# Ekumen-OS/beluga

Hardware: AMD Instinct MI355X
Metric: MCL update cycles/sec (motion+sensor+resample), N particles x 1080 beams (higher is better)
Workload: dtype f64; 1 GPU; BASELINE configs[1]: 1M particles/GPU, 1080-beam LikelihoodFieldModel, 4000x4000@5cm grid (seed 42), DifferentialDriveModel, multinomial resample every cycle; particles_per_gpu=1000000, particles_total=1000000, beams=1080, grid=4000x4000@0.05, parallelism=1 GPU

## Files before the change

### beluga_amd/csrc/context.hip

```cpp
#include <hip/hip_runtime.h>
#include <dlfcn.h>

#include <algorithm>
#include <cctype>
#include <atomic>
#include <chrono>
#include <thread>
#include <cmath>
#include <cstdio>
#include <cstring>
#include <limits>
#include <new>
#include <numeric>
#include <optional>
#include <string>
#include <unordered_set>
#include <map>
#include <vector>

#include "beluga_mcl.h"
#include "cluster_host.h"
#include "cycle_host.h"
#include "kernels.h"
#include "landmark_host.h"
// ... 1054 lines not shown
  const double* d_total = ctx->d_scalars.ptr + kSlotCdfTotal;
  uint64_t result = max_p;
  if (a.min_particles >= max_p) {
    ra.first_candidate = 0;
    ra.count = max_p;
    ra.out_offset = 0;
    if (opt.with_estimate) {
      MCL_HIP(ctx, ctx->d_est_partials.ensure(static_cast<size_t>(9) * ((max_p + 1023) / 1024)));
      Completion done{};
      const bool spin = ctx->tuning.cycle_spin > 0 || (ctx->tuning.cycle_spin < 0 && max_p >= 262144);
      ctx->done_armed = spin && ctx->profile <= 1 && opt.estimate_enqueued;
      if (ctx->done_armed) {
        done.d_ticket = reinterpret_cast<unsigned long long*>(ctx->d_scalars.ptr + kSlotDoneTicket);
        done.host_flag = reinterpret_cast<unsigned long long*>(ctx->hd_scalars + kSlotDoneWord);
        done.seq = ++ctx->done_seq;
      }
      const bool noise_in_draw = ctx->tuning.noise_ahead == 1 && max_p > 65536 && max_p <= 2000000 &&
                                 ctx->d_noise.ensure(3 * static_cast<size_t>(max_p)) == hipSuccess;
      const bool noise_ahead = ctx->done_armed && ctx->tuning.noise_ahead == 2 && max_p > 65536 && max_p <= 2000000 &&
                               ctx->d_noise.ensure(3 * static_cast<size_t>(max_p)) == hipSuccess;
      KeyFrame ahead_frame{};
      const bool order_keys = noise_in_draw && ctx->done_armed && ctx->tuning.order_ahead != 0 && max_p < (1ull << 32) && ctx->wants_ordering() &&
                              ctx->predict_key_frame(&ctx->last_sampler, &ahead_frame, 2);
      launch_resample_draw_and_estimate(ctx->stream, ctx->cur(), ctx->cdf_tree(), d_total, ctx->other(), ra, gv, fc, hp,
                                        ctx->facts.pivot()[0], ctx->facts.pivot()[1], ctx->d_est_partials.ptr, ctx->d_scalars.ptr + kSlotEstimate,
                                        ctx->hd_scalars + kSlotEstimate, ctx->done_armed ? &done : nullptr,
                                        ((ctx->tuning.draw_fold == 2 || (ctx->tuning.draw_fold == 1 && max_p <= 65536)) && ctx->d_scan_state.ptr)
                                            ? reinterpret_cast<unsigned int*>(ctx->d_scan_state.ptr + 4)
                                            : nullptr,
                                        noise_in_draw ? ctx->d_noise.ptr : nullptr, max_p, ctx->cfg.shard_offset, step + 1,
                                        order_keys ? ctx->sort_scratch().keys : nullptr, &ctx->last_sampler, &ahead_frame);
      if (noise_ahead) launch_noise_ahead(ctx->stream, ctx->cfg.seed, step + 1, ctx->cfg.shard_offset, max_p, ctx->d_noise.ptr);
      if (noise_ahead || noise_in_draw) ctx->facts.noise_ahead_recorded(step + 1, max_p, ctx->cfg.shard_offset, ctx->cfg.seed);
      if (order_keys) {
        const SortScratch sort = ctx->sort_scratch();
        launch_order_ahead(ctx->stream, max_p, &sort);
        ctx->facts.order_ahead_recorded(step + 1, max_p, ctx->key_layout());
        ctx->order_sampler = ctx->last_sampler;
      }
      if (opt.estimate_enqueued) *opt.estimate_enqueued = true;
    } else {
      launch_resample_draw(ctx->stream, ctx->cur(), ctx->cdf_tree(), d_total, ctx->other(), ra, gv, fc, hp, nullptr);
    }
    MCL_HIP(ctx, hipGetLastError());
  } else {
    MCL_REQUIRE(ctx, max_p < 0xFFFFFFFFull, "max_particles too large for KLD resampling");
    if (const mcl_status s = kld_begin(ctx)) return s;
    uint64_t chunk = std::max<uint64_t>(a.min_particles + 1, 1ull << 16);
    while (ctx->kld_pos < max_p) {
      const uint64_t pos = ctx->kld_pos;
      const uint64_t cnt = std::min(chunk, max_p - pos);
      if (const mcl_status s = kld_grow_table(ctx, pos + cnt)) return s;
      ra.first_candidate = pos;
      ra.count = cnt;
      ra.out_offset = pos;
      launch_resample_draw(ctx->stream, ctx->cur(), ctx->cdf_tree(), d_total, ctx->other(), ra, gv, fc, hp, ctx->d_hashes.ptr);
      uint64_t first_fail = ~0ull;
      if (const mcl_status s = kld_process(ctx, cnt, &first_fail)) return s;
      if (first_fail != ~0ull) {
// ... 948 lines not shown
      MCL_HIP(ctx, hipStreamCreateWithFlags(&ctx->stream, hipStreamNonBlocking));
      ctx->own_stream = true;
    }
    const uint64_t cap = cfg->shard_capacity ? cfg->shard_capacity : cfg->amcl.max_particles;
    if (const mcl_status s = ensure_capacity(ctx, cap)) return s;
    MCL_HIP(ctx, ctx->d_scalars.ensure(kScalarSlots));
    MCL_HIP(ctx, hipMemsetAsync(ctx->d_scalars.ptr, 0, kScalarSlots * sizeof(double), ctx->stream));
    MCL_HIP(ctx, hipHostMalloc(reinterpret_cast<void**>(&ctx->h_scalars), kScalarSlots * sizeof(double), hipHostMallocMapped));
    std::memset(ctx->h_scalars, 0, kScalarSlots * sizeof(double));
    MCL_HIP(ctx, hipHostGetDevicePointer(reinterpret_cast<void**>(&ctx->hd_scalars), ctx->h_scalars, 0));
    MCL_HIP(ctx, ctx->d_kld_scalars.ensure(8));
    MCL_HIP(ctx, hipMemsetAsync(ctx->d_kld_scalars.ptr, 0, 8 * sizeof(unsigned long long), ctx->stream));
    MCL_HIP(ctx, hipHostMalloc(reinterpret_cast<void**>(&ctx->h_kld_scalars), 8 * sizeof(unsigned long long)));
    for (auto& pair : ctx->ev)
      for (auto& e : pair) MCL_HIP(ctx, hipEventCreate(&e));
    MCL_HIP(ctx, hipEventCreateWithFlags(&ctx->points_event, hipEventDisableTiming));
    MCL_HIP(ctx, configure_device_kernels());
    {
      int count = 0;
      if (hipDeviceGetAttribute(&count, hipDeviceAttributeMultiprocessorCount, ctx->device) != hipSuccess || count <= 0) count = 256;
      ctx->tuning.device_cus = count;
    }
    for (const char* name : {"lf_variant", "lf_fast", "lf_table", "lf_patch", "lf_dispersed", "lf_far_tiles", "key_layout", "lf_loose_below", "lf_small_particles", "device_policy",
                             "sort_min_particles", "beam_sort_min_particles", "field_build", "key_curve", "key_warp", "key_bits_xy", "lf_margin", "lf_split", "lf_queue_grid", "shard_pad_permille", "lf_queue", "lf_ends_first", "beam_free_ahead", "beam_sectors", "lf_weight_sums", "beam_table", "cycle_spin", "scan_fused", "draw_fold", "lf_unit_weights", "small_fused", "norm_store", "noise_ahead", "order_ahead", "lf_far_beams_per_wave", "batch_cluster_fused"}) {
      std::string env = "BELUGA_MCL_";
      for (const char* c = name; *c; ++c) env += static_cast<char>(std::toupper(static_cast<unsigned char>(*c)));
      if (const char* v = std::getenv(env.c_str())) {
        if (std::string(name) == "lf_table") (void)mcl_set_option(ctx, name, std::string(v) == "cube" ? 1 : std::atoi(v));
        else (void)mcl_set_option(ctx, name, std::atoi(v));
      }
    }
    return MCL_OK;
  };
  st = init();
  if (st != MCL_OK) {
    g_create_error = ctx->error;
    mcl_destroy(ctx);
    return st;
  }
  *out = ctx;
  return MCL_OK;
}

void mcl_destroy(mcl_ctx* ctx) {
  if (!ctx || ctx->batch) return;
  drop_pending_map(ctx);
  (void)hipSetDevice(ctx->device);
// ... 1374 lines not shown
      t.shard_pad_permille = before;
      return s;
    }
  }
  else if (key == "lf_queue_grid") t.lf_queue_grid = static_cast<int>(std::clamp<int64_t>(value, 0, 1 << 20));
  else if (key == "cycle_spin") t.cycle_spin = value < 0 ? -1 : (value ? 1 : 0);
  else if (key == "beam_table") {
    t.beam_table = value ? 1 : 0;
    if (!t.beam_table && ctx->beam_table_ready) {
      if (bind_device(ctx) == MCL_OK && hipStreamSynchronize(ctx->stream) == hipSuccess) {
        ctx->d_beam_table.release();
        ctx->beam_table_ready = false;
      }
    }
  }
  else if (key == "lf_weight_sums") t.lf_weight_sums = value ? 1 : 0;
  else if (key == "scan_fused") t.scan_fused = static_cast<int>(std::clamp<int64_t>(value, 0, 2));
  else if (key == "draw_fold") t.draw_fold = static_cast<int>(std::clamp<int64_t>(value, 0, 2));
  else if (key == "lf_unit_weights") t.lf_unit_weights = value ? 1 : 0;
  else if (key == "small_fused") t.small_fused = value ? 1 : 0;
  else if (key == "batch_cluster_fused") t.batch_cluster_fused = value ? 1 : 0;
  else if (key == "norm_store") t.norm_store = value ? 1 : 0;
  else if (key == "order_ahead") t.order_ahead = value ? 1 : 0;
  else if (key == "noise_ahead") t.noise_ahead = static_cast<int>(std::clamp<int64_t>(value, 0, 2));
  else if (key == "lf_split") t.lf_split = static_cast<int>(value & 3);
  else if (key == "sort_min_particles") t.sort_min_particles = static_cast<int>(std::clamp<int64_t>(value, 0, 1ll << 30));
  else if (key == "beam_sort_min_particles") t.beam_sort_min_particles = static_cast<int>(std::clamp<int64_t>(value, 0, 1ll << 30));
  else return fail(ctx, MCL_ERR_INVALID_ARGUMENT, "mcl_set_option: unknown option " + key);
  return MCL_OK;
}

mcl_status mcl_get_counter(mcl_ctx* ctx, const char* name, uint64_t* value) {
  if (!ctx || !name || !value) return MCL_ERR_INVALID_ARGUMENT;
  const std::string key(name);
  if (key == "lf_fast_launches") *value = ctx->lf_fast_launches;
  else if (key == "lf_patch_launches") *value = ctx->lf_patch_launches;
  else if (key == "lf_queue_launches") *value = ctx->lf_queue_launches;
  else if (key == "lf_beams_launches") *value = ctx->lf_beams_launches;
  else if (key == "lf_far_launches") *value = ctx->lf_far_launches;
  else if (key == "lf_far_beams_launches") *value = ctx->lf_far_beams_launches;
  else if (key == "small_tail_launches") *value = ctx->small_tail_launches;
  else if (key == "estimate_repivots") *value = ctx->estimate_repivots;
  else if (key == "lf_far_tiles") *value = ctx->map->far_tiles;
  else if (key == "noise_ahead_used") *value = ctx->noise_ahead_used;
  else if (key == "order_ahead_used") *value = ctx->order_ahead_used;
  else if (key == "order_ahead_missed") *value = ctx->order_ahead_missed;
// ... 343 lines not shown
```

### beluga_amd/csrc/cycle_types.h

```cpp
#pragma once

#include <algorithm>
#include <cstdint>

namespace mcl {

struct DiffDriveSampler {
  int kind;
  double m1, s1, mt, st, m2, s2;
  double first_c, first_s;
};

enum LfVariant : int {
  kLfWavePerParticle = 0,
  kLfLanePerParticle = 1,
  kLfSortedLanes = 2,
  kLfBeamLanes = 3
};

struct Tuning {
  int lf_variant = kLfSortedLanes;
  int lf_fast = -1;
  int lf_table = 0;
  int lf_patch = 1;
// ... 6 lines not shown
  int lf_far_tiles = 1;
  int key_layout = -1;
  int lf_small_particles = 65536;
  int field_build = 0;
  int key_curve = 1;
  int key_warp = 1;
  int key_bits_xy = 0;
  int cycle_spin = -1;
  int beam_table = 1;
  int lf_weight_sums = 1;
  int lf_split = 3;
  int lf_margin = 1;
  int beam_free_ahead = 1;
  int lf_queue_grid = 0;
  int device_cus = 0;
  int shard_pad_permille = 1063;
  int lf_ends_first = 1;
  int beam_sectors = 1;
  int lf_queue = 1;
  int scan_fused = 1;
  int draw_fold = 1;
  int noise_ahead = 1;
  int order_ahead = 1;
  int norm_store = 0;
  int batch_cluster_fused = 1;
  int small_fused = 1;
  int lf_unit_weights = 1;
};

struct KeyFrame {
  double cx, cy;
  double c0, s0;
  float inv_x, inv_y;
  float inv_t, t_off;
  uint32_t layout;
  uint32_t bits_xy;
};

inline bool lf_set_is_small(uint64_t n, const Tuning& t) {
  return n < static_cast<uint64_t>(std::max(t.sort_min_particles, t.lf_small_particles));
}

}
```

### beluga_amd/csrc/kernels.h

```cpp
#pragma once
#include <hip/hip_runtime.h>

#include <algorithm>
#include <cstdint>

#include "batch_host.h"
#include "cycle_types.h"
#include "se2.h"
#include "sensor_records.h"

namespace mcl {

struct Particles {
  double4* pose;
  double* w;
};

struct FieldView {
  const float* data;
  uint32_t W, H;
  double inv_resolution;
  Pose2 world_to_field;
  float unknown_value;
  const double* cube;
// ... 168 lines not shown
  }
}
struct SortScratch {
  uint32_t* keys;
  uint32_t* perm;
  uint32_t* table;
  uint32_t* totals;
  unsigned long long* keyidx;
  double* bbox;
  KeyFrame* frame;
  double* partial;
};
constexpr uint32_t kLfMaxSegments = 16;
constexpr uint64_t kLfSegmentedBelow = 262144;

void launch_propagate(hipStream_t st, Particles p, uint64_t n, DiffDriveSampler smp, uint64_t seed, uint32_t step,
                      uint64_t index_offset, const double* scan_src = nullptr, double* scan_dst = nullptr, uint32_t scan_doubles = 0,
                      const SortScratch* sort = nullptr, const KeyFrame* frame = nullptr, const double* normals_ahead = nullptr,
                      uint64_t normals_stride = 0);
void launch_noise_ahead(hipStream_t st, uint64_t seed, uint32_t step, uint64_t index_offset, uint64_t n, double* d_normals);
void launch_pull_scan(hipStream_t st, const double* scan_src, double* scan_dst, uint32_t scan_doubles);
void launch_order_particles(hipStream_t st, Particles p, uint64_t n, const SortScratch* sort, const KeyFrame* frame, bool keys_ready,
                            uint32_t layout = 0);
void launch_order_ahead(hipStream_t st, uint64_t n, const SortScratch* sort);
struct PatchStats {
  unsigned long long* device;
  unsigned long long* mirror;
  uint32_t loose_below;
  uint32_t isotropic_margin;
  uint32_t split_patches;
  double* weight_sums;
  unsigned int* arrivals;
};
struct LfReweightArgs {
  Particles p;
  uint64_t n;
  FieldView f;
  const double* d_points;
  uint32_t B;
  const SortScratch* sort;
  bool patches, beams;
  bool dispersed;
  double scan_cells;
  bool unit_weights;
  PatchStats stats;
};
enum class LfKernel { kNone, kPatch, kPatchQueue, kFarBeams, kPaletteFar, kPaletteFast, kPaletteExact, kSortedCube, kSortedField, kBeams, kIndexOrder };
// ... 141 lines not shown
  unsigned long long done_seq;
};
SmallTailArgs small_tail_args(const SmallTail& t);
bool small_tail_fits(uint64_t n, uint64_t max_particles);

struct BatchItem {
  Particles p;
  uint64_t n;
  DiffDriveSampler smp;
  uint64_t seed;
  uint32_t step;
  uint64_t index_offset;
  const double* scan_src;
  double* scan_dst;
  uint32_t scan_doubles;
  FieldView f;
  uint32_t B;
  SmallTailArgs tail;
  uint32_t first_propagate_block, first_reweight_block;
};
void launch_batch_cycle(hipStream_t st, const BatchItem* d_items, const BatchGrid& grid);
void launch_resample_draw(hipStream_t st, Particles src, CdfTree cdf, const double* d_total, Particles dst,
                          ResampleArgs a, GridView g, FreeCells fc, HashParams hp, unsigned long long* d_hashes);
void launch_resample_draw_and_estimate(hipStream_t st, Particles src, CdfTree cdf, const double* d_total, Particles dst, ResampleArgs a,
                                       GridView g, FreeCells fc, HashParams hp, double pivot_x, double pivot_y, double* d_partials,
                                       double* d_sums, double* host_mirror, const Completion* done = nullptr,
                                       unsigned int* fold_ticket = nullptr, double* normals_ahead = nullptr, uint64_t normals_stride = 0,
                                       uint64_t normals_index_offset = 0, uint32_t normals_step = 0, uint32_t* keys_ahead = nullptr,
                                       const DiffDriveSampler* predicted = nullptr, const KeyFrame* frame_ahead = nullptr);
void launch_resample_targets(hipStream_t st, uint64_t seed, uint32_t step, double p, double total, uint64_t first_slot,
                             uint64_t count, uint64_t n_free, double* d_targets, const double* d_plan = nullptr);
struct RecoveryPolicy;
void launch_shard_plan(hipStream_t st, const double* d_stats, uint32_t world, uint64_t n_total, double* d_sums, double* sums_mirror,
                       const RecoveryPolicy& policy, double* d_intervals, double* d_plan);
void launch_route_targets(hipStream_t st, const double* d_targets, uint64_t count, const double* d_ends, const double* d_offsets,
                          uint32_t world, uint32_t self_rank, uint8_t* d_dest, uint32_t* d_block_hist, uint32_t* d_chunk_sum,
                          uint32_t* d_chunk_off, double* d_send_targets, uint32_t* d_order, long long* d_counts, uint32_t pad_capacity = 0,
                          double* d_overflow = nullptr);
void launch_gather_by_cdf_aos(hipStream_t st, Particles src, CdfTree cdf, const double* d_targets, uint64_t m,
                              double* d_out);
void launch_commit_routed(hipStream_t st, Particles dst, uint64_t seed, uint32_t step, uint64_t first_slot, uint64_t count,
                          const double* d_replies, const uint32_t* d_order, const double* d_targets, GridView g, FreeCells fc);
void launch_commit_injected(hipStream_t st, Particles dst, uint64_t seed, uint32_t step, uint64_t first_slot, uint64_t count,
                            const double* d_targets, GridView g, FreeCells fc);
void launch_finish_candidates(hipStream_t st, uint64_t seed, uint32_t step, uint64_t first_slot, uint64_t count, const double* d_replies,
                              const uint32_t* d_order, const double* d_targets, GridView g, FreeCells fc, HashParams hp,
                              double* d_states, unsigned long long* d_hashes);
struct KldTable {
  unsigned long long* keys;
  unsigned int* first;
  uint64_t capacity;
};
// ... 82 lines not shown
```

### beluga_amd/csrc/kernels.hip

```cpp
#include "device_common.hpp"


namespace mcl {
namespace {

constexpr uint32_t kKeyBitsXY = 6, kKeyBitsTheta = 8, kKeyBits = 2 * kKeyBitsXY + kKeyBitsTheta;
constexpr uint32_t kDigitBits = 10;
static_assert((1u << kDigitBits) == kSortDigits && kKeyBits == 2 * kDigitBits, "two passes of one digit each");
__device__ __forceinline__ uint32_t spread3(uint32_t v) {
  v &= 0x3FF;
  v = (v | (v << 16)) & 0x030000FF;
  v = (v | (v << 8)) & 0x0300F00F;
  v = (v | (v << 4)) & 0x030C30C3;
  v = (v | (v << 2)) & 0x09249249;
  return v;
}
__device__ __forceinline__ uint32_t spread2(uint32_t v) {
  v &= 0x3F;
  v = (v | (v << 4)) & 0x30F;
  v = (v | (v << 2)) & 0x333;
  v = (v | (v << 1)) & 0x555;
  return v;
}
__device__ __forceinline__ int unit_bin(float u, int bins) {
// ... 1447 lines not shown
      const uint32_t key = order_key(p.pose[i], kf);
      keys[i] = key;
      atomicAdd(&hist[key >> kDigitBits], 1u);
    }
  }
  __syncthreads();
  for (uint32_t d = threadIdx.x; d < kSortDigits; d += kWide) table[static_cast<size_t>(d) * nblocks + blockIdx.x] = hist[d];
}

__global__ __launch_bounds__(kWide) void k_key_hist(const uint32_t* __restrict__ keys, uint64_t n, uint32_t* __restrict__ table, uint32_t nblocks) {
  __shared__ uint32_t hist[kSortDigits];
  for (uint32_t d = threadIdx.x; d < kSortDigits; d += kWide) hist[d] = 0;
  __syncthreads();
  const uint64_t base = static_cast<uint64_t>(blockIdx.x) * kChunk;
#pragma unroll
  for (int k = 0; k < kChunk / kWide; ++k) {
    const uint64_t i = base + k * kWide + threadIdx.x;
    if (i < n) atomicAdd(&hist[keys[i] >> kDigitBits], 1u);
  }
  __syncthreads();
  for (uint32_t d = threadIdx.x; d < kSortDigits; d += kWide) table[static_cast<size_t>(d) * nblocks + blockIdx.x] = hist[d];
}

__global__ __launch_bounds__(kBlock) void k_row_scan(uint32_t* __restrict__ table, uint32_t nblocks, uint32_t* __restrict__ totals) {
  const uint32_t d = blockIdx.x * (kBlock / 64) + (threadIdx.x >> 6), lane = threadIdx.x & 63;
  uint32_t* row = table + static_cast<size_t>(d) * nblocks;
  uint32_t carry = 0;
  for (uint32_t start = 0; start < nblocks; start += 64) {
    const uint32_t b = start + lane;
    const uint32_t v = b < nblocks ? row[b] : 0u;
    uint32_t incl = v;
#pragma unroll
    for (int o = 1; o < 64; o <<= 1) {
      const uint32_t up = __shfl_up(incl, o);
      if (lane >= static_cast<uint32_t>(o)) incl += up;
    }
    if (b < nblocks) row[b] = carry + incl - v;
    carry += __shfl(incl, 63);
  }
  if (lane == 0) totals[d] = carry;
}
template <int T>
__device__ __forceinline__ void digit_bases(const uint32_t* __restrict__ totals, uint32_t* s_base, uint32_t* s_wave ) {
  constexpr int kPer = kSortDigits / T;
  const uint32_t lane = threadIdx.x & 63, wave = threadIdx.x >> 6;
  uint32_t v[kPer], sum = 0;
#pragma unroll
  for (int k = 0; k < kPer; ++k) {
    v[k] = totals[threadIdx.x * kPer + k];
    sum += v[k];
  }
  uint32_t incl = sum;
#pragma unroll
  for (int o = 1; o < 64; o <<= 1) {
    const uint32_t up = __shfl_up(incl, o);
    if (lane >= static_cast<uint32_t>(o)) incl += up;
  }
  if (lane == 63) s_wave[wave] = incl;
  __syncthreads();
  uint32_t prefix = incl - sum;
  for (uint32_t q = 0; q < wave; ++q) prefix += s_wave[q];
#pragma unroll
  for (int k = 0; k < kPer; ++k) {
// ... 294 lines not shown
      if (base + e < n) a[base + e] = lds[chunk_slot(e)];
    }
  }
}

__global__ __launch_bounds__(kBlock) void k_chunk_sum(const double* __restrict__ w, uint64_t n, double* __restrict__ partials) {
  __shared__ double scratch[kBlock / 64];
  __shared__ double s_items[kChunkPadded];
  double x[kItems];
  chunk_items_load(w, n, s_items, x);
  double v[1] = {0.0};
#pragma unroll
  for (int k = 0; k < kItems; ++k) v[0] += x[k];
  block_reduce<1>(v, scratch);
  if (threadIdx.x == 0) partials[blockIdx.x] = v[0];
}

__device__ __forceinline__ double row_total(const double* __restrict__ row, uint32_t count, double* scratch ) {
  double v[1] = {0.0};
  for (uint32_t b = threadIdx.x; b < count; b += kBlock) v[0] += row[b];
  block_reduce<1>(v, scratch);
  return v[0];
}
__global__ __launch_bounds__(kBlock) void k_final_rows(const double* __restrict__ partials, uint32_t count, uint32_t stride,
                                                       double* __restrict__ out, double* __restrict__ host_mirror, Completion done) {
  __shared__ double scratch[kBlock / 64];
  const uint32_t k = blockIdx.x;
  const double total = row_total(partials + static_cast<size_t>(k) * stride, count, scratch);
  if (threadIdx.x == 0) {
    out[k] = total;
    if (host_mirror) host_mirror[k] = total;
    if (done.host_flag) {
      __threadfence_system();
      const unsigned long long ticket = atomicAdd(done.d_ticket, 1ull);
      if (ticket % gridDim.x == gridDim.x - 1) {
        __threadfence_system();
        __hip_atomic_store(done.host_flag, done.seq, __ATOMIC_RELEASE, __HIP_MEMORY_SCOPE_SYSTEM);
      }
    }
  }
}

__global__ __launch_bounds__(kBlock) void k_normalize(double* __restrict__ w, uint64_t n, const double* __restrict__ d_factor,
                                                      double* __restrict__ chunk_sum, double* __restrict__ chunk_sumsq,
                                                      const double* __restrict__ sum_partials, uint32_t sum_count,
                                                      double* __restrict__ d_sum_out, double* __restrict__ sum_mirror, int store_weights) {
  __shared__ double scratch[(kBlock / 64) * 2];
  __shared__ double s_factor;
  if (sum_partials) {
    double t[1] = {0.0};
    for (uint32_t b = threadIdx.x; b < sum_count; b += kBlock) t[0] += sum_partials[b];
    block_reduce<1>(t, scratch);
    if (threadIdx.x == 0) {
      s_factor = t[0];
      if (blockIdx.x == 0) {
        d_sum_out[0] = t[0];
        if (sum_mirror) sum_mirror[0] = t[0];
      }
    }
    __syncthreads();
  }
  const double factor = sum_partials ? s_factor : *d_factor;
  const bool skip = fabs(factor - 1.0) < DBL_EPSILON;
// ... 515 lines not shown
  return s;
}

__device__ __forceinline__ bool intersperse_here(const RngWords& r, uint64_t j, double p, uint64_t n_free) {
  return j > 0 && p > 0.0 && rng_uniform32(r.w[2]) < p && n_free > 0;
}

constexpr int kDrawBlock = 1024;
constexpr uint32_t kDrawStageMax = 4608;
struct DrawFold {
  unsigned int* ticket{nullptr};
  double* out{nullptr};
  double* host_mirror{nullptr};
  Completion done{};
};
struct DrawNormals {
  double* normals{nullptr};
  uint64_t stride{0};
  uint64_t index_offset{0};
  uint32_t step{0};
  uint32_t* keys{nullptr};
  DiffDriveSampler predicted{};
  KeyFrame frame{};
};
__device__ __forceinline__ double4 predicted_pose_f32(const Pose2& p, const DiffDriveSampler& m, float z0, float z1, float z2) {
  const float c = static_cast<float>(p.r.c), s = static_cast<float>(p.r.s);
  float turn, ahead, left, dir_c, dir_s;
  if (m.kind == 1) {
    turn = z0 * static_cast<float>(m.s1) + static_cast<float>(m.m1);
    ahead = z1 * static_cast<float>(m.st) + static_cast<float>(m.mt);
    left = -(z2 * static_cast<float>(m.s2));
    dir_c = static_cast<float>(m.first_c);
    dir_s = static_cast<float>(m.first_s);
  } else if (m.kind == 2) {
    turn = z0 * 0.02f;
    ahead = z1 * 0.02f;
    left = z2 * 0.02f;
    dir_c = 1.f;
    dir_s = 0.f;
  } else {
    const float r1 = z0 * static_cast<float>(m.s1) + static_cast<float>(m.m1);
    turn = r1 + z2 * static_cast<float>(m.s2) + static_cast<float>(m.m2);
    ahead = z1 * static_cast<float>(m.st) + static_cast<float>(m.mt);
    left = 0.f;
    dir_c = __cosf(r1);
    dir_s = __sinf(r1);
  }
  const float hc = c * dir_c - s * dir_s, hs = s * dir_c + c * dir_s;
  const float tc = __cosf(turn), ts = __sinf(turn);
  return double4{static_cast<double>(c * tc - s * ts), static_cast<double>(s * tc + c * ts),
                 p.x + static_cast<double>(ahead * hc - left * hs), p.y + static_cast<double>(ahead * hs + left * hc)};
}
template <bool kEstimate>
__global__ __launch_bounds__(kDrawBlock) __attribute__((amdgpu_waves_per_eu(8, 8))) void k_resample_draw(Particles src, CdfTree cdf, const double* __restrict__ d_total,
                                                              Particles dst, ResampleArgs a, GridView g, FreeCells fc, HashParams hp,
                                                              unsigned long long* __restrict__ hashes, double pivot_x, double pivot_y,
                                                              double* __restrict__ est_partials, uint32_t est_stride, int first_staged,
                                                              uint32_t staged_doubles, DrawFold fold, DrawNormals ahead) {
  extern __shared__ __attribute__((aligned(16))) unsigned char smem[];
  double* staged = reinterpret_cast<double*>(smem);
  __shared__ double scratch[kEstimate ? (kDrawBlock / 64) * 9 : 1];
  if (first_staged < cdf.depth) {
    const double* from = cdf.levels + cdf.offset[first_staged];
    for (uint32_t k = threadIdx.x; k < staged_doubles; k += kDrawBlock) staged[k] = from[k];
  }
  __syncthreads();
  const uint64_t t = static_cast<uint64_t>(blockIdx.x) * kDrawBlock + threadIdx.x;
  double v[9] = {0, 0, 0, 0, 0, 0, 0, 0, 0};
  const uint64_t j = a.first_candidate + t;
  const RngWords r = rng_draw(a.seed, a.step, kRngResample, j);
  const double p_random = a.d_random_state_probability ? *a.d_random_state_probability : a.random_state_probability;
  const bool intersperse = t < a.count && intersperse_here(r, j, p_random, fc.count);
  uint64_t idx = 0;
  if (a.n_in >= 2) {
    const double target = (t < a.count && !intersperse) ? rng_uniform53(r.w[0], r.w[1]) * (*d_total) : 0.0;
    idx = cdf_tree_lower_bound_staged(cdf, staged, first_staged, target);
  }
  if (t < a.count) {
    Pose2 s;
    if (intersperse) {
      s = random_free_state(a.seed, a.step, j, g, fc);
    } else {
      s = load_pose(src, idx);
    }
    const uint64_t o = a.out_offset + t;
    store_pose(dst, o, s);
    dst.w[o] = 1.0;
    if (hashes) hashes[o] = spatial_hash(s, hp);
    if (ahead.normals) {
      const double4 z = propagation_normals(a.seed, ahead.step, ahead.index_offset + o);
      ahead.normals[o] = z.x;
      ahead.normals[ahead.stride + o] = z.y;
      ahead.normals[2 * ahead.stride + o] = z.z;
      if (ahead.keys)
        ahead.keys[o] = order_key(predicted_pose_f32(s, ahead.predicted, static_cast<float>(z.x), static_cast<float>(z.y), static_cast<float>(z.z)),
                                  ahead.frame);
    }
    if (kEstimate) {
      const double dx = s.x - pivot_x, dy = s.y - pivot_y;
      v[0] = 1.0;
      v[1] = 1.0;
      v[2] = s.r.c;
      v[3] = s.r.s;
      v[4] = dx;
      v[5] = dy;
      v[6] = dx * dx;
      v[7] = dx * dy;
      v[8] = dy * dy;
    }
  }
  if (kEstimate) {
    block_reduce<9, kDrawBlock>(v, scratch);
    if (fold.ticket == nullptr) {
      if (threadIdx.x == 0) {
#pragma unroll
        for (int k = 0; k < 9; ++k) est_partials[static_cast<size_t>(k) * est_stride + blockIdx.x] = v[k];
      }
      return;
    }
    __shared__ uint32_t s_last;
    if (threadIdx.x == 0) {
#pragma unroll
      for (int k = 0; k < 9; ++k)
        __hip_atomic_store(est_partials + static_cast<size_t>(k) * est_stride + blockIdx.x, v[k], __ATOMIC_RELAXED, __HIP_MEMORY_SCOPE_AGENT);
      asm volatile("s_waitcnt vmcnt(0)" ::: "memory");
      s_last = atomicInc(fold.ticket, gridDim.x - 1u) == gridDim.x - 1u ? 1u : 0u;
    }
    __syncthreads();
    if (s_last == 0u) return;
    const uint32_t group = threadIdx.x >> 8, t = threadIdx.x & 255u, wave_in_group = t >> 6;
    double* group_scratch = scratch + group * 4;
#pragma unroll 1
    for (uint32_t round = 0; round < 3; ++round) {
      const uint32_t k = round * 4 + group;
      double acc = 0.0;
// ... 1205 lines not shown
}

void launch_pull_scan(hipStream_t st, const double* scan_src, double* scan_dst, uint32_t scan_doubles) {
  if (scan_doubles == 0) return;
  hipLaunchKernelGGL(k_pull_scan, dim3(1), dim3(kBlock), 0, st, scan_src, scan_dst, scan_doubles);
}

void launch_order_particles(hipStream_t st, Particles p, uint64_t n, const SortScratch* sort, const KeyFrame* frame, bool keys_ready,
                            uint32_t layout) {
  if (n == 0 || !sort || n >= (1ull << 32)) return;
  const uint32_t nblocks = num_chunks(n);
  if (!keys_ready) {
    const KeyFrame* device_frame = nullptr;
    if (!frame) {
      double* partials = sort->bbox + 8;
      hipLaunchKernelGGL(k_bbox_partials, dim3(nblocks), dim3(kBlock), 0, st, p, n, partials, nblocks);
      hipLaunchKernelGGL(k_bbox_final, dim3(1), dim3(kBlock), 0, st, partials, nblocks, nblocks, sort->bbox, p, sort->frame, layout);
      device_frame = sort->frame;
    }
    hipLaunchKernelGGL(k_order_keys, dim3(nblocks), dim3(kWide), 0, st, p, n, frame ? *frame : KeyFrame{}, device_frame, sort->keys,
                       sort->table, nblocks);
  }
  const dim3 rows(kSortDigits / (kBlock / 64));
  hipLaunchKernelGGL(k_row_scan, rows, dim3(kBlock), 0, st, sort->table, nblocks, sort->totals);
  hipLaunchKernelGGL(k_sort_scatter_high, dim3(nblocks), dim3(kStable), 0, st, sort->keys, n, sort->table, nblocks, sort->totals,
                     sort->keyidx, sort->totals + kSortDigits);
  hipLaunchKernelGGL(k_sort_buckets, dim3(kSortDigits), dim3(kStable), 0, st, sort->keyidx, sort->totals, sort->totals + kSortDigits,
                     sort->perm);
}

void launch_order_ahead(hipStream_t st, uint64_t n, const SortScratch* sort) {
  if (n == 0 || !sort || n >= (1ull << 32)) return;
  const uint32_t nblocks = num_chunks(n);
  hipLaunchKernelGGL(k_key_hist, dim3(nblocks), dim3(kWide), 0, st, sort->keys, n, sort->table, nblocks);
  const dim3 rows(kSortDigits / (kBlock / 64));
  hipLaunchKernelGGL(k_row_scan, rows, dim3(kBlock), 0, st, sort->table, nblocks, sort->totals);
  hipLaunchKernelGGL(k_sort_scatter_high, dim3(nblocks), dim3(kStable), 0, st, sort->keys, n, sort->table, nblocks, sort->totals,
                     sort->keyidx, sort->totals + kSortDigits);
  hipLaunchKernelGGL(k_sort_buckets, dim3(kSortDigits), dim3(kStable), 0, st, sort->keyidx, sort->totals, sort->totals + kSortDigits,
                     sort->perm);
}

namespace {
constexpr uint32_t kFarBeamsMaxLds = 80 * 1024;
uint32_t far_beams_points_at(const FieldView& f) {
  return (kFarBeamsPalShift + f.pal_base + f.pal_count * 8u + 15u) & ~15u;
}
uint32_t far_beams_lds(const FieldView& f, uint32_t B) {
  return far_beams_points_at(f) + ((B + 63u) & ~63u) * 16u + (kFarBeamsBlock / kWave) * kFarBeamsChunk * 32u;
}
}

hipError_t configure_device_kernels() {
  const struct { const void* kernel; size_t lds; } opt_ins[] = {
      {reinterpret_cast<const void*>(k_reweight_lf_far_beams<false>), kFarBeamsMaxLds},
      {reinterpret_cast<const void*>(k_reweight_lf_far_beams<true>), kFarBeamsMaxLds},
      {reinterpret_cast<const void*>(k_small_tail), kSmallLdsBytes},
      {reinterpret_cast<const void*>(k_batch_small_tail), kSmallLdsBytes},
      {reinterpret_cast<const void*>(k_small_cluster_cells), kSmallClusterLdsBytes},
// ... 241 lines not shown

namespace {
void draw_staging(const CdfTree& t, int& first, uint32_t& doubles) {
  first = t.depth;
  doubles = 0;
  while (first > 0 && t.offset[t.depth - 1] + t.size[t.depth - 1] - t.offset[first - 1] <= kDrawStageMax) {
    --first;
    doubles = t.offset[t.depth - 1] + t.size[t.depth - 1] - t.offset[first];
  }
}
}

void launch_resample_draw(hipStream_t st, Particles src, CdfTree cdf, const double* d_total, Particles dst,
                          ResampleArgs a, GridView g, FreeCells fc, HashParams hp, unsigned long long* d_hashes) {
  if (a.count == 0) return;
  int first;
  uint32_t doubles;
  draw_staging(cdf, first, doubles);
  const unsigned blocks = static_cast<unsigned>((a.count + kDrawBlock - 1) / kDrawBlock);
  hipLaunchKernelGGL(k_resample_draw<false>, dim3(blocks), dim3(kDrawBlock), doubles * sizeof(double), st, src, cdf, d_total, dst, a, g,
                     fc, hp, d_hashes, 0.0, 0.0, static_cast<double*>(nullptr), 0u, first, doubles, DrawFold{}, DrawNormals{});
}

void launch_resample_draw_and_estimate(hipStream_t st, Particles src, CdfTree cdf, const double* d_total, Particles dst, ResampleArgs a,
                                       GridView g, FreeCells fc, HashParams hp, double pivot_x, double pivot_y, double* d_partials,
                                       double* d_sums, double* host_mirror, const Completion* done, unsigned int* fold_ticket,
                                       double* normals_ahead, uint64_t normals_stride, uint64_t normals_index_offset, uint32_t normals_step,
                                       uint32_t* keys_ahead, const DiffDriveSampler* predicted, const KeyFrame* frame_ahead) {
  int first;
  uint32_t doubles;
  draw_staging(cdf, first, doubles);
  const unsigned blocks = static_cast<unsigned>((a.count + kDrawBlock - 1) / kDrawBlock);
  const bool fold = fold_ticket != nullptr && blocks > 0 && blocks <= 4096u;
  if (blocks) {
    DrawFold f{};
    if (fold) f = DrawFold{fold_ticket, d_sums, host_mirror, done ? *done : Completion{}};
    hipLaunchKernelGGL(k_resample_draw<true>, dim3(blocks), dim3(kDrawBlock), doubles * sizeof(double), st, src, cdf, d_total, dst, a, g,
                       fc, hp, static_cast<unsigned long long*>(nullptr), pivot_x, pivot_y, d_partials, blocks, first, doubles, f,
                       DrawNormals{normals_ahead, normals_stride, normals_index_offset, normals_step,
                                   (normals_ahead && predicted && frame_ahead) ? keys_ahead : nullptr,
                                   predicted ? *predicted : DiffDriveSampler{}, frame_ahead ? *frame_ahead : KeyFrame{}});
  }
  if (!fold)
    hipLaunchKernelGGL(k_final_rows, dim3(9), dim3(kBlock), 0, st, d_partials, blocks, blocks, d_sums, host_mirror, done ? *done : Completion{});
}

void launch_resample_targets(hipStream_t st, uint64_t seed, uint32_t step, double p, double total, uint64_t first_slot,
                             uint64_t count, uint64_t n_free, double* d_targets, const double* d_plan) {
  if (count == 0) return;
  hipLaunchKernelGGL(k_resample_targets, dim3(blocks_for(count)), dim3(kBlock), 0, st, seed, step, p, total, first_slot, count, n_free,
                     d_targets, d_plan);
}

__global__ void k_shard_plan(const double* __restrict__ stats, uint32_t world, NormFinalize fin, double* __restrict__ intervals,
                             double* __restrict__ d_plan) {
  if (threadIdx.x != 0) return;
  double run = 0.0, norm_sum = 0.0, norm_sumsq = 0.0;
  for (uint32_t r = 0; r < world; ++r) {
    intervals[world + r] = run;
    run += stats[3 * r];
    intervals[r] = run;
    norm_sum += stats[3 * r + 1];
    norm_sumsq += stats[3 * r + 2];
  }
  fin.d_sums[0] = norm_sum;
  fin.d_sums[1] = norm_sumsq;
  if (fin.sums_mirror) {
// ... 272 lines not shown
```

Baseline: 1621 cycles/s.

## Fold sort key histogram into resample draw and merge row scan with final rows

The resample draw kernel now builds a per-workgroup LDS histogram of the high digit of the look-ahead order keys and writes it to scratch. This removes the separate key histogram pass over the keys before the ordering sort. Optionally the row scan that turns these half-column histograms into a prefix table is merged into the final-rows reduction launch, saving another kernel launch. The cost is LDS atomics in the draw kernel, extra scratch writes, and reuse of the keyidx buffer to hold the half histograms.

```diff
diff --git a/beluga_amd/csrc/context.hip b/beluga_amd/csrc/context.hip
--- a/beluga_amd/csrc/context.hip
+++ b/beluga_amd/csrc/context.hip
@@ -1100,19 +1100,20 @@
       KeyFrame ahead_frame{};
       const bool order_keys = noise_in_draw && ctx->done_armed && ctx->tuning.order_ahead != 0 && max_p < (1ull << 32) && ctx->wants_ordering() &&
                               ctx->predict_key_frame(&ctx->last_sampler, &ahead_frame, 2);
-      launch_resample_draw_and_estimate(ctx->stream, ctx->cur(), ctx->cdf_tree(), d_total, ctx->other(), ra, gv, fc, hp,
+      const SortScratch ahead_sort = order_keys ? ctx->sort_scratch() : SortScratch{};
+      const OrderAheadDone order_done = launch_resample_draw_and_estimate(ctx->stream, ctx->cur(), ctx->cdf_tree(), d_total, ctx->other(), ra, gv, fc, hp,
                                         ctx->facts.pivot()[0], ctx->facts.pivot()[1], ctx->d_est_partials.ptr, ctx->d_scalars.ptr + kSlotEstimate,
                                         ctx->hd_scalars + kSlotEstimate, ctx->done_armed ? &done : nullptr,
                                         ((ctx->tuning.draw_fold == 2 || (ctx->tuning.draw_fold == 1 && max_p <= 65536)) && ctx->d_scan_state.ptr)
                                             ? reinterpret_cast<unsigned int*>(ctx->d_scan_state.ptr + 4)
                                             : nullptr,
                                         noise_in_draw ? ctx->d_noise.ptr : nullptr, max_p, ctx->cfg.shard_offset, step + 1,
-                                        order_keys ? ctx->sort_scratch().keys : nullptr, &ctx->last_sampler, &ahead_frame);
+                                        order_keys ? ahead_sort.keys : nullptr, &ctx->last_sampler, &ahead_frame,
+                                        (order_keys && ctx->tuning.draw_key_hist) ? &ahead_sort : nullptr, ctx->tuning.rows_merged != 0);
       if (noise_ahead) launch_noise_ahead(ctx->stream, ctx->cfg.seed, step + 1, ctx->cfg.shard_offset, max_p, ctx->d_noise.ptr);
       if (noise_ahead || noise_in_draw) ctx->facts.noise_ahead_recorded(step + 1, max_p, ctx->cfg.shard_offset, ctx->cfg.seed);
       if (order_keys) {
-        const SortScratch sort = ctx->sort_scratch();
-        launch_order_ahead(ctx->stream, max_p, &sort);
+        launch_order_ahead(ctx->stream, max_p, &ahead_sort, order_done);
         ctx->facts.order_ahead_recorded(step + 1, max_p, ctx->key_layout());
         ctx->order_sampler = ctx->last_sampler;
       }
@@ -2107,7 +2108,7 @@
       ctx->tuning.device_cus = count;
     }
     for (const char* name : {"lf_variant", "lf_fast", "lf_table", "lf_patch", "lf_dispersed", "lf_far_tiles", "key_layout", "lf_loose_below", "lf_small_particles", "device_policy",
-                             "sort_min_particles", "beam_sort_min_particles", "field_build", "key_curve", "key_warp", "key_bits_xy", "lf_margin", "lf_split", "lf_queue_grid", "shard_pad_permille", "lf_queue", "lf_ends_first", "beam_free_ahead", "beam_sectors", "lf_weight_sums", "beam_table", "cycle_spin", "scan_fused", "draw_fold", "lf_unit_weights", "small_fused", "norm_store", "noise_ahead", "order_ahead", "lf_far_beams_per_wave", "batch_cluster_fused"}) {
+                             "sort_min_particles", "beam_sort_min_particles", "field_build", "key_curve", "key_warp", "key_bits_xy", "lf_margin", "lf_split", "lf_queue_grid", "shard_pad_permille", "lf_queue", "lf_ends_first", "beam_free_ahead", "beam_sectors", "lf_weight_sums", "beam_table", "cycle_spin", "scan_fused", "draw_fold", "lf_unit_weights", "small_fused", "norm_store", "noise_ahead", "order_ahead", "lf_far_beams_per_wave", "batch_cluster_fused", "draw_key_hist", "rows_merged"}) {
       std::string env = "BELUGA_MCL_";
       for (const char* c = name; *c; ++c) env += static_cast<char>(std::toupper(static_cast<unsigned char>(*c)));
       if (const char* v = std::getenv(env.c_str())) {
@@ -3528,6 +3529,8 @@
   else if (key == "batch_cluster_fused") t.batch_cluster_fused = value ? 1 : 0;
   else if (key == "norm_store") t.norm_store = value ? 1 : 0;
   else if (key == "order_ahead") t.order_ahead = value ? 1 : 0;
+  else if (key == "draw_key_hist") t.draw_key_hist = value ? 1 : 0;
+  else if (key == "rows_merged") t.rows_merged = value ? 1 : 0;
   else if (key == "noise_ahead") t.noise_ahead = static_cast<int>(std::clamp<int64_t>(value, 0, 2));
   else if (key == "lf_split") t.lf_split = static_cast<int>(value & 3);
   else if (key == "sort_min_particles") t.sort_min_particles = static_cast<int>(std::clamp<int64_t>(value, 0, 1ll << 30));
diff --git a/beluga_amd/csrc/cycle_types.h b/beluga_amd/csrc/cycle_types.h
--- a/beluga_amd/csrc/cycle_types.h
+++ b/beluga_amd/csrc/cycle_types.h
@@ -52,6 +52,8 @@
   int draw_fold = 1;
   int noise_ahead = 1;
   int order_ahead = 1;
+  int draw_key_hist = 1;
+  int rows_merged = 1;
   int norm_store = 0;
   int batch_cluster_fused = 1;
   int small_fused = 1;
diff --git a/beluga_amd/csrc/kernels.h b/beluga_amd/csrc/kernels.h
--- a/beluga_amd/csrc/kernels.h
+++ b/beluga_amd/csrc/kernels.h
@@ -214,7 +214,12 @@
 void launch_pull_scan(hipStream_t st, const double* scan_src, double* scan_dst, uint32_t scan_doubles);
 void launch_order_particles(hipStream_t st, Particles p, uint64_t n, const SortScratch* sort, const KeyFrame* frame, bool keys_ready,
                             uint32_t layout = 0);
-void launch_order_ahead(hipStream_t st, uint64_t n, const SortScratch* sort);
+enum OrderAheadDone : int {
+  kOrderAheadKeys = 0,
+  kOrderAheadHalfColumns = 1,
+  kOrderAheadTable = 2
+};
+void launch_order_ahead(hipStream_t st, uint64_t n, const SortScratch* sort, OrderAheadDone done = kOrderAheadKeys);
 struct PatchStats {
   unsigned long long* device;
   unsigned long long* mirror;
@@ -402,12 +407,14 @@
 void launch_batch_cycle(hipStream_t st, const BatchItem* d_items, const BatchGrid& grid);
 void launch_resample_draw(hipStream_t st, Particles src, CdfTree cdf, const double* d_total, Particles dst,
                           ResampleArgs a, GridView g, FreeCells fc, HashParams hp, unsigned long long* d_hashes);
-void launch_resample_draw_and_estimate(hipStream_t st, Particles src, CdfTree cdf, const double* d_total, Particles dst, ResampleArgs a,
-                                       GridView g, FreeCells fc, HashParams hp, double pivot_x, double pivot_y, double* d_partials,
-                                       double* d_sums, double* host_mirror, const Completion* done = nullptr,
-                                       unsigned int* fold_ticket = nullptr, double* normals_ahead = nullptr, uint64_t normals_stride = 0,
-                                       uint64_t normals_index_offset = 0, uint32_t normals_step = 0, uint32_t* keys_ahead = nullptr,
-                                       const DiffDriveSampler* predicted = nullptr, const KeyFrame* frame_ahead = nullptr);
+OrderAheadDone launch_resample_draw_and_estimate(hipStream_t st, Particles src, CdfTree cdf, const double* d_total, Particles dst, ResampleArgs a,
+                                                 GridView g, FreeCells fc, HashParams hp, double pivot_x, double pivot_y, double* d_partials,
+                                                 double* d_sums, double* host_mirror, const Completion* done = nullptr,
+                                                 unsigned int* fold_ticket = nullptr, double* normals_ahead = nullptr,
+                                                 uint64_t normals_stride = 0, uint64_t normals_index_offset = 0, uint32_t normals_step = 0,
+                                                 uint32_t* keys_ahead = nullptr, const DiffDriveSampler* predicted = nullptr,
+                                                 const KeyFrame* frame_ahead = nullptr, const SortScratch* hist_sort = nullptr,
+                                                 bool rows_merged = false);
 void launch_resample_targets(hipStream_t st, uint64_t seed, uint32_t step, double p, double total, uint64_t first_slot,
                              uint64_t count, uint64_t n_free, double* d_targets, const double* d_plan = nullptr);
 struct RecoveryPolicy;
diff --git a/beluga_amd/csrc/kernels.hip b/beluga_amd/csrc/kernels.hip
--- a/beluga_amd/csrc/kernels.hip
+++ b/beluga_amd/csrc/kernels.hip
@@ -1493,13 +1493,22 @@
   for (uint32_t d = threadIdx.x; d < kSortDigits; d += kWide) table[static_cast<size_t>(d) * nblocks + blockIdx.x] = hist[d];
 }
 
-__global__ __launch_bounds__(kBlock) void k_row_scan(uint32_t* __restrict__ table, uint32_t nblocks, uint32_t* __restrict__ totals) {
-  const uint32_t d = blockIdx.x * (kBlock / 64) + (threadIdx.x >> 6), lane = threadIdx.x & 63;
+__device__ __forceinline__ void row_scan_rows(uint32_t block, uint32_t* __restrict__ table, uint32_t nblocks, uint32_t* __restrict__ totals,
+                                              const uint32_t* __restrict__ halves, uint32_t nhalves) {
+  const uint32_t d = block * (kBlock / 64) + (threadIdx.x >> 6), lane = threadIdx.x & 63;
   uint32_t* row = table + static_cast<size_t>(d) * nblocks;
   uint32_t carry = 0;
   for (uint32_t start = 0; start < nblocks; start += 64) {
     const uint32_t b = start + lane;
-    const uint32_t v = b < nblocks ? row[b] : 0u;
+    uint32_t v = 0u;
+    if (b < nblocks) {
+      if (halves) {
+        const uint32_t* first = halves + static_cast<size_t>(2u * b) * kSortDigits + d;
+        v = (2u * b < nhalves ? first[0] : 0u) + (2u * b + 1u < nhalves ? first[kSortDigits] : 0u);
+      } else {
+        v = row[b];
+      }
+    }
     uint32_t incl = v;
 #pragma unroll
     for (int o = 1; o < 64; o <<= 1) {
@@ -1510,6 +1519,10 @@
     carry += __shfl(incl, 63);
   }
   if (lane == 0) totals[d] = carry;
+}
+__global__ __launch_bounds__(kBlock) void k_row_scan(uint32_t* __restrict__ table, uint32_t nblocks, uint32_t* __restrict__ totals,
+                                                     const uint32_t* __restrict__ halves, uint32_t nhalves) {
+  row_scan_rows(blockIdx.x, table, nblocks, totals, halves, nhalves);
 }
 template <int T>
 __device__ __forceinline__ void digit_bases(const uint32_t* __restrict__ totals, uint32_t* s_base, uint32_t* s_wave ) {
@@ -1850,10 +1863,8 @@
   block_reduce<1>(v, scratch);
   return v[0];
 }
-__global__ __launch_bounds__(kBlock) void k_final_rows(const double* __restrict__ partials, uint32_t count, uint32_t stride,
-                                                       double* __restrict__ out, double* __restrict__ host_mirror, Completion done) {
-  __shared__ double scratch[kBlock / 64];
-  const uint32_t k = blockIdx.x;
+__device__ __forceinline__ void final_row(uint32_t k, uint32_t rows, const double* __restrict__ partials, uint32_t count, uint32_t stride,
+                                          double* __restrict__ out, double* __restrict__ host_mirror, const Completion& done, double* scratch) {
   const double total = row_total(partials + static_cast<size_t>(k) * stride, count, scratch);
   if (threadIdx.x == 0) {
     out[k] = total;
@@ -1861,12 +1872,27 @@
     if (done.host_flag) {
       __threadfence_system();
       const unsigned long long ticket = atomicAdd(done.d_ticket, 1ull);
-      if (ticket % gridDim.x == gridDim.x - 1) {
+      if (ticket % rows == rows - 1) {
         __threadfence_system();
         __hip_atomic_store(done.host_flag, done.seq, __ATOMIC_RELEASE, __HIP_MEMORY_SCOPE_SYSTEM);
       }
     }
   }
+}
+__global__ __launch_bounds__(kBlock) void k_final_rows(const double* __restrict__ partials, uint32_t count, uint32_t stride,
+                                                       double* __restrict__ out, double* __restrict__ host_mirror, Completion done) {
+  __shared__ double scratch[kBlock / 64];
+  final_row(blockIdx.x, gridDim.x, partials, count, stride, out, host_mirror, done, scratch);
+}
+__global__ __launch_bounds__(kBlock) void k_final_rows_row_scan(uint32_t rows, const double* __restrict__ partials, uint32_t count, uint32_t stride,
+                                                                double* __restrict__ out, double* __restrict__ host_mirror, Completion done,
+                                                                uint32_t* __restrict__ table, uint32_t nblocks, uint32_t* __restrict__ totals,
+                                                                const uint32_t* __restrict__ halves, uint32_t nhalves) {
+  __shared__ double scratch[kBlock / 64];
+  if (blockIdx.x < rows)
+    final_row(blockIdx.x, rows, partials, count, stride, out, host_mirror, done, scratch);
+  else
+    row_scan_rows(blockIdx.x - rows, table, nblocks, totals, halves, nhalves);
 }
 
 __global__ __launch_bounds__(kBlock) void k_normalize(double* __restrict__ w, uint64_t n, const double* __restrict__ d_factor,
@@ -2428,7 +2454,9 @@
   uint32_t* keys{nullptr};
   DiffDriveSampler predicted{};
   KeyFrame frame{};
+  uint32_t* half_hist{nullptr};
 };
+static_assert(kDrawBlock == static_cast<int>(kSortDigits) && kChunk == 2 * kDrawBlock, "a thread per digit counter; two draw workgroups per chunk");
 __device__ __forceinline__ double4 predicted_pose_f32(const Pose2& p, const DiffDriveSampler& m, float z0, float z1, float z2) {
   const float c = static_cast<float>(p.r.c), s = static_cast<float>(p.r.s);
   float turn, ahead, left, dir_c, dir_s;
@@ -2466,6 +2494,8 @@
   extern __shared__ __attribute__((aligned(16))) unsigned char smem[];
   double* staged = reinterpret_cast<double*>(smem);
   __shared__ double scratch[kEstimate ? (kDrawBlock / 64) * 9 : 1];
+  __shared__ uint32_t key_hist[kEstimate ? kSortDigits : 1];
+  if (kEstimate && ahead.half_hist) key_hist[threadIdx.x] = 0u;
   if (first_staged < cdf.depth) {
     const double* from = cdf.levels + cdf.offset[first_staged];
     for (uint32_t k = threadIdx.x; k < staged_doubles; k += kDrawBlock) staged[k] = from[k];
@@ -2498,9 +2528,12 @@
       ahead.normals[o] = z.x;
       ahead.normals[ahead.stride + o] = z.y;
       ahead.normals[2 * ahead.stride + o] = z.z;
-      if (ahead.keys)
-        ahead.keys[o] = order_key(predicted_pose_f32(s, ahead.predicted, static_cast<float>(z.x), static_cast<float>(z.y), static_cast<float>(z.z)),
-                                  ahead.frame);
+      if (ahead.keys) {
+        const uint32_t key = order_key(predicted_pose_f32(s, ahead.predicted, static_cast<float>(z.x), static_cast<float>(z.y), static_cast<float>(z.z)),
+                                       ahead.frame);
+        ahead.keys[o] = key;
+        if (kEstimate && ahead.half_hist) atomicAdd(&key_hist[key >> kDigitBits], 1u);
+      }
     }
     if (kEstimate) {
       const double dx = s.x - pivot_x, dy = s.y - pivot_y;
@@ -2517,6 +2550,8 @@
   }
   if (kEstimate) {
     block_reduce<9, kDrawBlock>(v, scratch);
+    if (ahead.half_hist)
+      ahead.half_hist[static_cast<size_t>(blockIdx.x) * kSortDigits + threadIdx.x] = key_hist[threadIdx.x];
     if (fold.ticket == nullptr) {
       if (threadIdx.x == 0) {
 #pragma unroll
@@ -3768,19 +3803,29 @@
                        sort->table, nblocks);
   }
   const dim3 rows(kSortDigits / (kBlock / 64));
-  hipLaunchKernelGGL(k_row_scan, rows, dim3(kBlock), 0, st, sort->table, nblocks, sort->totals);
+  hipLaunchKernelGGL(k_row_scan, rows, dim3(kBlock), 0, st, sort->table, nblocks, sort->totals, static_cast<const uint32_t*>(nullptr), 0u);
   hipLaunchKernelGGL(k_sort_scatter_high, dim3(nblocks), dim3(kStable), 0, st, sort->keys, n, sort->table, nblocks, sort->totals,
                      sort->keyidx, sort->totals + kSortDigits);
   hipLaunchKernelGGL(k_sort_buckets, dim3(kSortDigits), dim3(kStable), 0, st, sort->keyidx, sort->totals, sort->totals + kSortDigits,
                      sort->perm);
 }
 
-void launch_order_ahead(hipStream_t st, uint64_t n, const SortScratch* sort) {
+namespace {
+uint32_t* order_half_columns(const SortScratch* sort) { return reinterpret_cast<uint32_t*>(sort->keyidx); }
+uint32_t draw_workgroups(uint64_t n) { return static_cast<uint32_t>((n + kDrawBlock - 1) / kDrawBlock); }
+}
+
+void launch_order_ahead(hipStream_t st, uint64_t n, const SortScratch* sort, OrderAheadDone done) {
   if (n == 0 || !sort || n >= (1ull << 32)) return;
   const uint32_t nblocks = num_chunks(n);
-  hipLaunchKernelGGL(k_key_hist, dim3(nblocks), dim3(kWide), 0, st, sort->keys, n, sort->table, nblocks);
   const dim3 rows(kSortDigits / (kBlock / 64));
-  hipLaunchKernelGGL(k_row_scan, rows, dim3(kBlock), 0, st, sort->table, nblocks, sort->totals);
+  if (done == kOrderAheadKeys) {
+    hipLaunchKernelGGL(k_key_hist, dim3(nblocks), dim3(kWide), 0, st, sort->keys, n, sort->table, nblocks);
+    hipLaunchKernelGGL(k_row_scan, rows, dim3(kBlock), 0, st, sort->table, nblocks, sort->totals, static_cast<const uint32_t*>(nullptr), 0u);
+  } else if (done == kOrderAheadHalfColumns) {
+    hipLaunchKernelGGL(k_row_scan, rows, dim3(kBlock), 0, st, sort->table, nblocks, sort->totals,
+                       static_cast<const uint32_t*>(order_half_columns(sort)), draw_workgroups(n));
+  }
   hipLaunchKernelGGL(k_sort_scatter_high, dim3(nblocks), dim3(kStable), 0, st, sort->keys, n, sort->table, nblocks, sort->totals,
                      sort->keyidx, sort->totals + kSortDigits);
   hipLaunchKernelGGL(k_sort_buckets, dim3(kSortDigits), dim3(kStable), 0, st, sort->keyidx, sort->totals, sort->totals + kSortDigits,
@@ -4068,27 +4113,43 @@
                      fc, hp, d_hashes, 0.0, 0.0, static_cast<double*>(nullptr), 0u, first, doubles, DrawFold{}, DrawNormals{});
 }
 
-void launch_resample_draw_and_estimate(hipStream_t st, Particles src, CdfTree cdf, const double* d_total, Particles dst, ResampleArgs a,
-                                       GridView g, FreeCells fc, HashParams hp, double pivot_x, double pivot_y, double* d_partials,
-                                       double* d_sums, double* host_mirror, const Completion* done, unsigned int* fold_ticket,
-                                       double* normals_ahead, uint64_t normals_stride, uint64_t normals_index_offset, uint32_t normals_step,
-                                       uint32_t* keys_ahead, const DiffDriveSampler* predicted, const KeyFrame* frame_ahead) {
+OrderAheadDone launch_resample_draw_and_estimate(hipStream_t st, Particles src, CdfTree cdf, const double* d_total, Particles dst, ResampleArgs a,
+                                                 GridView g, FreeCells fc, HashParams hp, double pivot_x, double pivot_y, double* d_partials,
+                                                 double* d_sums, double* host_mirror, const Completion* done, unsigned int* fold_ticket,
+                                                 double* normals_ahead, uint64_t normals_stride, uint64_t normals_index_offset,
+                                                 uint32_t normals_step, uint32_t* keys_ahead, const DiffDriveSampler* predicted,
+                                                 const KeyFrame* frame_ahead, const SortScratch* hist_sort, bool rows_merged) {
   int first;
   uint32_t doubles;
   draw_staging(cdf, first, doubles);
-  const unsigned blocks = static_cast<unsigned>((a.count + kDrawBlock - 1) / kDrawBlock);
+  const unsigned blocks = draw_workgroups(a.count);
+  uint32_t* const keys = (normals_ahead && predicted && frame_ahead) ? keys_ahead : nullptr;
+  const uint32_t nblocks = num_chunks(a.count);
+  const bool count_keys = keys && hist_sort && keys == hist_sort->keys && a.out_offset == 0 && a.count < (1ull << 32) &&
+                          static_cast<uint64_t>(kSortDigits) * 2u * nblocks <= 2u * a.count;
+  OrderAheadDone order = kOrderAheadKeys;
   const bool fold = fold_ticket != nullptr && blocks > 0 && blocks <= 4096u;
   if (blocks) {
     DrawFold f{};
     if (fold) f = DrawFold{fold_ticket, d_sums, host_mirror, done ? *done : Completion{}};
     hipLaunchKernelGGL(k_resample_draw<true>, dim3(blocks), dim3(kDrawBlock), doubles * sizeof(double), st, src, cdf, d_total, dst, a, g,
                        fc, hp, static_cast<unsigned long long*>(nullptr), pivot_x, pivot_y, d_partials, blocks, first, doubles, f,
-                       DrawNormals{normals_ahead, normals_stride, normals_index_offset, normals_step,
-                                   (normals_ahead && predicted && frame_ahead) ? keys_ahead : nullptr,
-                                   predicted ? *predicted : DiffDriveSampler{}, frame_ahead ? *frame_ahead : KeyFrame{}});
-  }
-  if (!fold)
-    hipLaunchKernelGGL(k_final_rows, dim3(9), dim3(kBlock), 0, st, d_partials, blocks, blocks, d_sums, host_mirror, done ? *done : Completion{});
+                       DrawNormals{normals_ahead, normals_stride, normals_index_offset, normals_step, keys,
+                                   predicted ? *predicted : DiffDriveSampler{}, frame_ahead ? *frame_ahead : KeyFrame{},
+                                   count_keys ? order_half_columns(hist_sort) : nullptr});
+    if (count_keys) order = kOrderAheadHalfColumns;
+  }
+  if (!fold) {
+    if (order == kOrderAheadHalfColumns && rows_merged) {
+      hipLaunchKernelGGL(k_final_rows_row_scan, dim3(9 + kSortDigits / (kBlock / 64)), dim3(kBlock), 0, st, 9u, d_partials, blocks, blocks, d_sums,
+                         host_mirror, done ? *done : Completion{}, hist_sort->table, nblocks, hist_sort->totals,
+                         static_cast<const uint32_t*>(order_half_columns(hist_sort)), blocks);
+      order = kOrderAheadTable;
+    } else {
+      hipLaunchKernelGGL(k_final_rows, dim3(9), dim3(kBlock), 0, st, d_partials, blocks, blocks, d_sums, host_mirror, done ? *done : Completion{});
+    }
+  }
+  return order;
 }
 
 void launch_resample_targets(hipStream_t st, uint64_t seed, uint32_t step, double p, double total, uint64_t first_slot,
```

Measured after the change: 1641 cycles/s, median of 6. 1.01x the previous value.
